# berkeley-hipie/HIPIE

Measured on AMD Instinct MI355X. Metric: images/sec @1024x1024 ViT-H bs=8 (single-image inference hot path: box, class and mask logits), higher is better.
Workload: dtype f16x3 (split-fp16 operands, fp32 accumulate: fp32-class); 1 GPU; BASELINE.json configs[2]: vit_huge, 1024x1024, batch 8 per GPU, 80 class prompts (L=194), detection; global_batch=8, parallelism=dp1, precision_policy=split, launch=eager

## Files before the change

hipie_amd/csrc/ffn_fused.hip:

```cpp
#include "common.h"
#include "mfma.h"
#include "wave.h"

namespace hipie {

struct FFParams {
  const char* X; const char* W1; const char* W2; const float* b1; const float* b2; float* out;
  long ldx_b, ldw1_b, ldw2_b, ldo;
  int M;
};

constexpr int FF_D = 256, FF_F = 2048, FF_C = 32;
constexpr int FF_W1B = FF_C * FF_D * 4;
constexpr int FF_W2B = FF_D * FF_C * 4;
constexpr int FF_BUF = FF_W1B + FF_W2B;

__global__ __launch_bounds__(256, 1) void ffn_fused_kernel(const FFParams p) {
  typedef f16_t T;
  typedef Mfma32<T>::frag frag;
  constexpr int KS = FF_D / 16;
  constexpr int NB = FF_D / 32;
  constexpr int NCH = FF_F / FF_C;
  extern __shared__ __attribute__((aligned(1024))) char smem[];
  float* sb1 = reinterpret_cast<float*>(smem + 2 * FF_BUF);

  const int tid = threadIdx.x, lane = tid & 63;
  const int wave = __builtin_amdgcn_readfirstlane(tid >> 6);
  const int li = lane & 31, hi = lane >> 5;
  const int m = blockIdx.x * 128 + wave * 32 + li;
  const int mc = min(m, p.M - 1);

  for (int i = tid; i < FF_F / 4; i += 256) reinterpret_cast<float4*>(sb1)[i] = reinterpret_cast<const float4*>(p.b1)[i];

  frag xh[KS], xl[KS];
  {
    const char* xr = p.X + (long)mc * p.ldx_b + 32 * hi;
#pragma unroll
    for (int ks = 0; ks < KS; ++ks) {
      xh[ks] = *reinterpret_cast<const frag*>(xr + 64 * ks);
      xl[ks] = *reinterpret_cast<const frag*>(xr + 64 * ks + 16);
    }
  }

  unsigned int dv1[8], dv2[8];
#pragma unroll
  for (int q = 0; q < 8; ++q) {
    const int i = wave + 4 * q;
    dv1[q] = (unsigned int)((long)i * p.ldw1_b + 16 * (lane ^ (i & 15)));
    const int f = 8 * i + (lane >> 3);
    dv2[q] = (unsigned int)((long)f * p.ldw2_b + 16 * ((lane & 7) ^ ((f >> 1) & 7)));
  }
  const unsigned int lds0 = (unsigned int)reinterpret_cast<uintptr_t>((__attribute__((address_space(3))) char*)smem);
  auto dma_chunk = [&](const int c, const int buf, const int q) {
    const int i = wave + 4 * q;
    dma16(p.W1 + (long)c * FF_C * p.ldw1_b, dv1[q], __builtin_amdgcn_readfirstlane(lds0 + (unsigned int)(buf * FF_BUF + 1024 * i)));
    dma16(p.W2 + (long)c * (FF_C * 4), dv2[q], __builtin_amdgcn_readfirstlane(lds0 + (unsigned int)(buf * FF_BUF + FF_W1B + 1024 * i)));
  };

  f32x16 acc[NB];
#pragma unroll
  for (int j = 0; j < NB; ++j)
#pragma unroll
    for (int r = 0; r < 16; ++r) acc[j][r] = 0.f;

#pragma unroll
  for (int q = 0; q < 8; ++q) dma_chunk(0, 0, q);

  const int w1row = li * 1024, w1sw = li & 15;
  const int w2row = FF_W1B + li * 128, w2sw = (li >> 1) & 7;

  for (int c = 0; c < NCH; ++c) {
    const int buf = c & 1;
    __builtin_amdgcn_s_waitcnt(vmcnt(0));
    __syncthreads();
    const char* bs = smem + buf * FF_BUF;
    const bool more = c + 1 < NCH;

    f32x16 h0, h1;
#pragma unroll
    for (int r = 0; r < 16; ++r) { h0[r] = 0.f; h1[r] = 0.f; }
#pragma unroll
    for (int ks = 0; ks < KS; ks += 2) {
      const frag ah0 = *reinterpret_cast<const frag*>(bs + w1row + 16 * ((2 * (2 * ks + hi)) ^ w1sw));
      const frag al0 = *reinterpret_cast<const frag*>(bs + w1row + 16 * ((2 * (2 * ks + hi) + 1) ^ w1sw));
      const frag ah1 = *reinterpret_cast<const frag*>(bs + w1row + 16 * ((2 * (2 * ks + 2 + hi)) ^ w1sw));
      const frag al1 = *reinterpret_cast<const frag*>(bs + w1row + 16 * ((2 * (2 * ks + 2 + hi) + 1) ^ w1sw));
      h0 = Mfma32<T>::mma(al0, xh[ks], h0);
      h1 = Mfma32<T>::mma(al1, xh[ks + 1], h1);
      h0 = Mfma32<T>::mma(ah0, xl[ks], h0);
      h1 = Mfma32<T>::mma(ah1, xl[ks + 1], h1);
      h0 = Mfma32<T>::mma(ah0, xh[ks], h0);
      h1 = Mfma32<T>::mma(ah1, xh[ks + 1], h1);
      if (more) dma_chunk(c + 1, buf ^ 1, ks >> 1);
    }
    frag Hh[2], Hl[2];
#pragma unroll
    for (int g = 0; g < 4; ++g) {
      const float4 b4 = *reinterpret_cast<const float4*>(sb1 + c * FF_C + 8 * g + 4 * hi);
      const float bb[4] = {b4.x, b4.y, b4.z, b4.w};
#pragma unroll
      for (int e = 0; e < 4; ++e) {
        const int r = 4 * g + e;
        T hh, ll;
        hl_split(fmaxf(h0[r] + h1[r] + bb[e], 0.f), hh, ll);
        Hh[r >> 3][r & 7] = hh;
        Hl[r >> 3][r & 7] = ll;
      }
    }
#pragma unroll
    for (int s2 = 0; s2 < 2; ++s2) {
      frag wh[NB], wl[NB];
#pragma unroll
      for (int j = 0; j < NB; ++j) {
        wh[j] = *reinterpret_cast<const frag*>(bs + w2row + j * 4096 + 16 * ((2 * (2 * s2 + hi)) ^ w2sw));
        wl[j] = *reinterpret_cast<const frag*>(bs + w2row + j * 4096 + 16 * ((2 * (2 * s2 + hi) + 1) ^ w2sw));
      }
#pragma unroll
      for (int j = 0; j < NB; ++j) acc[j] = Mfma32<T>::mma(wl[j], Hh[s2], acc[j]);
#pragma unroll
      for (int j = 0; j < NB; ++j) acc[j] = Mfma32<T>::mma(wh[j], Hl[s2], acc[j]);
#pragma unroll
      for (int j = 0; j < NB; ++j) acc[j] = Mfma32<T>::mma(wh[j], Hh[s2], acc[j]);
    }
  }

  if (m < p.M) {
    float* orow = p.out + (long)m * p.ldo;
#pragma unroll
    for (int j = 0; j < NB; ++j)
#pragma unroll
      for (int g = 0; g < 4; ++g) {
        const int n = 32 * j + 8 * g + 4 * hi;
        const float4 b4 = *reinterpret_cast<const float4*>(p.b2 + n);
        *reinterpret_cast<float4*>(orow + n) = make_float4(acc[j][4 * g] + b4.x, acc[j][4 * g + 1] + b4.y, acc[j][4 * g + 2] + b4.z, acc[j][4 * g + 3] + b4.w);
      }
  }
}

}

extern "C" int hipie_ffn_fused(const void* x, int64_t ldx, const void* w1, const float* b1, const void* w2p, const float* b2, float* out,
                               int64_t ldo, int M, int D, int F, void* stream) {
  using namespace hipie;
  HIPIE_REQUIRE(x && w1 && b1 && w2p && b2 && out, "ffn_fused: null pointer");
  HIPIE_REQUIRE(D == FF_D && F == FF_F, "ffn_fused: model width %d / hidden width %d (built for 256 / 2048)", D, F);
  HIPIE_REQUIRE(M > 0 && ldx >= 2 * D && ldx % 8 == 0 && ldo >= D && ldo % 4 == 0, "ffn_fused: M=%d ldx=%ld ldo=%ld", M, (long)ldx, (long)ldo);
  HIPIE_REQUIRE((((uintptr_t)x | (uintptr_t)w1 | (uintptr_t)w2p | (uintptr_t)b1 | (uintptr_t)b2 | (uintptr_t)out) & 15) == 0,
                "ffn_fused: pointers must be 16-byte aligned");
  FFParams p;
  p.X = (const char*)x; p.W1 = (const char*)w1; p.W2 = (const char*)w2p; p.b1 = b1; p.b2 = b2; p.out = out;
  p.ldx_b = ldx * 2; p.ldw1_b = (long)2 * D * 2; p.ldw2_b = (long)2 * F * 2; p.ldo = ldo;
  p.M = M;
  const size_t lds = (size_t)2 * FF_BUF + FF_F * sizeof(float);
  static LdsLimit limit;
  limit.raise((const void*)ffn_fused_kernel, lds);
  hipLaunchKernelGGL(ffn_fused_kernel, dim3((unsigned)((M + 127) / 128)), dim3(256), lds, (hipStream_t)stream, p);
  return check_launch("ffn_fused");
}
```

Before: 42.86 images/sec.

## Add 16x16 MFMA variant of fused FFN kernel with register double-buffered LDS fragments

Adds a second fused FFN kernel that uses 16x16x32 MFMA tiles instead of 32x32, with each wave covering two 16-row tiles. It changes the LDS swizzle and DMA row mapping to suit the new fragment layout, and software-pipelines W1/W2 fragment loads from LDS into double-buffered registers, using sched_barrier to order loads and MFMAs. The new kernel is the default, selectable through an environment variable. The aim is higher MFMA throughput and hiding LDS read latency, at the cost of more accumulator and fragment registers and a more intricate swizzle.

```diff
diff --git a/hipie_amd/csrc/ffn_fused.hip b/hipie_amd/csrc/ffn_fused.hip
--- a/hipie_amd/csrc/ffn_fused.hip
+++ b/hipie_amd/csrc/ffn_fused.hip
@@ -135,6 +135,173 @@
         *reinterpret_cast<float4*>(orow + n) = make_float4(acc[j][4 * g] + b4.x, acc[j][4 * g + 1] + b4.y, acc[j][4 * g + 2] + b4.z, acc[j][4 * g + 3] + b4.w);
       }
   }
+}
+
+__device__ __forceinline__ constexpr int ff_swz16(const int r) { return ((r >> 1) & 3) | (((((r & 15) + 4) >> 3) & 1) << 2); }
+
+__global__ __launch_bounds__(256, 1) void ffn_fused16_kernel(const FFParams p) {
+  typedef f16_t T;
+  typedef Mfma16<T>::frag frag;
+  constexpr int KS = FF_D / 32;
+  constexpr int NF = FF_D / 16;
+  constexpr int NCH = FF_F / FF_C;
+  extern __shared__ __attribute__((aligned(1024))) char smem[];
+  float* sb1 = reinterpret_cast<float*>(smem + 2 * FF_BUF);
+
+  const int tid = threadIdx.x, lane = tid & 63;
+  const int wave = __builtin_amdgcn_readfirstlane(tid >> 6);
+  const int lc = lane & 15, lg = lane >> 4;
+  const int m0 = blockIdx.x * 128 + wave * 32 + lc;
+
+  for (int i = tid; i < FF_F / 4; i += 256) reinterpret_cast<float4*>(sb1)[i] = reinterpret_cast<const float4*>(p.b1)[i];
+
+  frag xh[2][KS], xl[2][KS];
+#pragma unroll
+  for (int tb = 0; tb < 2; ++tb) {
+    const char* xr = p.X + (long)min(m0 + 16 * tb, p.M - 1) * p.ldx_b + 32 * lg;
+#pragma unroll
+    for (int ks = 0; ks < KS; ++ks) {
+      xh[tb][ks] = *reinterpret_cast<const frag*>(xr + 128 * ks);
+      xl[tb][ks] = *reinterpret_cast<const frag*>(xr + 128 * ks + 16);
+    }
+  }
+
+  unsigned int dv1[8], dv2[8];
+#pragma unroll
+  for (int q = 0; q < 8; ++q) {
+    const int i = wave + 4 * q;
+    const int u = (i & 7) + 8 * (i >> 4) + 16 * ((i >> 3) & 1);
+    dv1[q] = (unsigned int)((long)u * p.ldw1_b + 16 * (lane ^ (i & 15)));
+    const int f = 8 * i + (lane >> 3);
+    dv2[q] = (unsigned int)((long)f * p.ldw2_b + 16 * ((lane & 7) ^ ff_swz16(f)));
+  }
+  const unsigned int lds0 = (unsigned int)reinterpret_cast<uintptr_t>((__attribute__((address_space(3))) char*)smem);
+  auto dma_chunk = [&](const int c, const int buf, const int q) {
+    const int i = wave + 4 * q;
+    dma16(p.W1 + (long)c * FF_C * p.ldw1_b, dv1[q], __builtin_amdgcn_readfirstlane(lds0 + (unsigned int)(buf * FF_BUF + 1024 * i)));
+    dma16(p.W2 + (long)c * (FF_C * 4), dv2[q], __builtin_amdgcn_readfirstlane(lds0 + (unsigned int)(buf * FF_BUF + FF_W1B + 1024 * i)));
+  };
+
+  f32x4 acc[NF][2];
+#pragma unroll
+  for (int j = 0; j < NF; ++j)
+#pragma unroll
+    for (int tb = 0; tb < 2; ++tb)
+#pragma unroll
+      for (int r = 0; r < 4; ++r) acc[j][tb][r] = 0.f;
+
+#pragma unroll
+  for (int q = 0; q < 8; ++q) dma_chunk(0, 0, q);
+
+  int w1o[2][2], w2o[2];
+#pragma unroll
+  for (int lo = 0; lo < 2; ++lo) {
+#pragma unroll
+    for (int k1 = 0; k1 < 2; ++k1) w1o[lo][k1] = lc * 1024 + 16 * ((8 * k1 + 2 * lg + lo) ^ lc);
+    w2o[lo] = FF_W1B + lc * 128 + 16 * ((2 * lg + lo) ^ ff_swz16(lc));
+  }
+  const int b1o = ((4 * lg) & 7) + 16 * (lg >> 1);
+
+  for (int c = 0; c < NCH; ++c) {
+    const int buf = c & 1;
+    __builtin_amdgcn_s_waitcnt(vmcnt(0));
+    __syncthreads();
+    const char* bs = smem + buf * FF_BUF;
+    const bool more = c + 1 < NCH;
+    frag fr[2][4];
+    auto load_w1 = [&](const int ks) {
+#pragma unroll
+      for (int i = 0; i < 4; ++i)
+        fr[ks & 1][i] = *reinterpret_cast<const frag*>(bs + w1o[i >> 1][ks & 1] + 256 * (ks >> 1) + 16384 * (i & 1));
+    };
+    auto load_w2 = [&](const int s) {
+#pragma unroll
+      for (int i = 0; i < 4; ++i) fr[s & 1][i] = *reinterpret_cast<const frag*>(bs + w2o[i >> 1] + (2 * s + (i & 1)) * 2048);
+    };
+    load_w1(0);
+    float4 b4[2];
+#pragma unroll
+    for (int hb = 0; hb < 2; ++hb) b4[hb] = *reinterpret_cast<const float4*>(sb1 + c * FF_C + 8 * hb + b1o);
+
+    f32x4 h[2][2];
+#pragma unroll
+    for (int hb = 0; hb < 2; ++hb)
+#pragma unroll
+      for (int tb = 0; tb < 2; ++tb)
+#pragma unroll
+        for (int r = 0; r < 4; ++r) h[hb][tb][r] = 0.f;
+#pragma unroll
+    for (int ks = 0; ks < KS; ++ks) {
+      if (ks + 1 < KS) load_w1(ks + 1); else load_w2(0);
+      __builtin_amdgcn_sched_barrier(0);
+      const frag (&f)[4] = fr[ks & 1];
+#pragma unroll
+      for (int hb = 0; hb < 2; ++hb)
+#pragma unroll
+        for (int tb = 0; tb < 2; ++tb) h[hb][tb] = Mfma16<T>::mma(f[2 + hb], xh[tb][ks], h[hb][tb]);
+#pragma unroll
+      for (int hb = 0; hb < 2; ++hb)
+#pragma unroll
+        for (int tb = 0; tb < 2; ++tb) h[hb][tb] = Mfma16<T>::mma(f[hb], xl[tb][ks], h[hb][tb]);
+#pragma unroll
+      for (int hb = 0; hb < 2; ++hb)
+#pragma unroll
+        for (int tb = 0; tb < 2; ++tb) h[hb][tb] = Mfma16<T>::mma(f[hb], xh[tb][ks], h[hb][tb]);
+      if (more) dma_chunk(c + 1, buf ^ 1, ks);
+    }
+    frag Hh[2], Hl[2];
+#pragma unroll
+    for (int hb = 0; hb < 2; ++hb) {
+      const float bb[4] = {b4[hb].x, b4[hb].y, b4[hb].z, b4[hb].w};
+#pragma unroll
+      for (int tb = 0; tb < 2; ++tb)
+#pragma unroll
+        for (int r = 0; r < 4; ++r) {
+          T hh, ll;
+          hl_split(fmaxf(h[hb][tb][r] + bb[r], 0.f), hh, ll);
+          Hh[tb][4 * hb + r] = hh;
+          Hl[tb][4 * hb + r] = ll;
+        }
+    }
+#pragma unroll
+    for (int s = 0; s < NF / 2; ++s) {
+      if (s + 1 < NF / 2) load_w2(s + 1);
+      __builtin_amdgcn_sched_barrier(0);
+      const frag (&f)[4] = fr[s & 1];
+#pragma unroll
+      for (int j = 0; j < 2; ++j)
+#pragma unroll
+        for (int tb = 0; tb < 2; ++tb) acc[2 * s + j][tb] = Mfma16<T>::mma(f[2 + j], Hh[tb], acc[2 * s + j][tb]);
+#pragma unroll
+      for (int j = 0; j < 2; ++j)
+#pragma unroll
+        for (int tb = 0; tb < 2; ++tb) acc[2 * s + j][tb] = Mfma16<T>::mma(f[j], Hl[tb], acc[2 * s + j][tb]);
+#pragma unroll
+      for (int j = 0; j < 2; ++j)
+#pragma unroll
+        for (int tb = 0; tb < 2; ++tb) acc[2 * s + j][tb] = Mfma16<T>::mma(f[j], Hh[tb], acc[2 * s + j][tb]);
+      __builtin_amdgcn_sched_barrier(0);
+    }
+  }
+
+#pragma unroll
+  for (int tb = 0; tb < 2; ++tb) {
+    const int m = m0 + 16 * tb;
+    if (m < p.M) {
+      float* orow = p.out + (long)m * p.ldo + 4 * lg;
+#pragma unroll
+      for (int j = 0; j < NF; ++j) {
+        const float4 b4 = *reinterpret_cast<const float4*>(p.b2 + 16 * j + 4 * lg);
+        *reinterpret_cast<float4*>(orow + 16 * j) =
+            make_float4(acc[j][tb][0] + b4.x, acc[j][tb][1] + b4.y, acc[j][tb][2] + b4.z, acc[j][tb][3] + b4.w);
+      }
+    }
+  }
+}
+
+static inline bool ffn_mfma16() {
+  const char* e = study_env("HIPIE_FFN_MFMA");
+  return e ? atoi(e) == 16 : true;
 }
 
 }
@@ -152,8 +319,13 @@
   p.ldx_b = ldx * 2; p.ldw1_b = (long)2 * D * 2; p.ldw2_b = (long)2 * F * 2; p.ldo = ldo;
   p.M = M;
   const size_t lds = (size_t)2 * FF_BUF + FF_F * sizeof(float);
-  static LdsLimit limit;
-  limit.raise((const void*)ffn_fused_kernel, lds);
-  hipLaunchKernelGGL(ffn_fused_kernel, dim3((unsigned)((M + 127) / 128)), dim3(256), lds, (hipStream_t)stream, p);
+  static LdsLimit limit, limit16;
+  if (ffn_mfma16()) {
+    limit16.raise((const void*)ffn_fused16_kernel, lds);
+    hipLaunchKernelGGL(ffn_fused16_kernel, dim3((unsigned)((M + 127) / 128)), dim3(256), lds, (hipStream_t)stream, p);
+  } else {
+    limit.raise((const void*)ffn_fused_kernel, lds);
+    hipLaunchKernelGGL(ffn_fused_kernel, dim3((unsigned)((M + 127) / 128)), dim3(256), lds, (hipStream_t)stream, p);
+  }
   return check_launch("ffn_fused");
 }
```

After: 43.27 images/sec (median of 6 runs). About the same (+1.0%).
